# biodatageeks/datafusion-bio-functions

Hardware: AMD Instinct MI355X
Metric: overlap-pairs/sec + probe-rows/sec, IntervalJoinExec 100Mx1M (higher is better)
Workload: dtype int32; 1 GPU; join_100Mx1M_24contigs; probe_rows_per_gpu=100000000, build_rows_per_gpu=1000000, contigs=24, pairs_per_gpu=37210484, parallelism=partition-per-gpu x1, gather=False, build_overlap=True

## Files before the change

datafusion-bio-functions_amd/csrc/ivx_capi.hip:

```cpp
#include "ivx_internal.hpp"
#include <cstdlib>
#include <atomic>
#include <chrono>
#include <cstring>
#include <mutex>
#include <new>
#include <thread>
#include <condition_variable>
#include <deque>


void ivx_ctx::join_tail()
{
    if (!tail_pending) return;
    (void)hipStreamWaitEvent(stream, tail_ev, 0);
    tail_pending = false;
}

ivx_status ivx_ctx::get_scratch(int slot, size_t bytes, void **out)
{
    if (tail_pending && slot != WS_SORTHIST && slot != WS_T0 && slot != WS_T1 && slot != WS_T2) join_tail();
    ivx_buf &b = scratch[slot];
    if (sub_plan.valid && ((sub_plan.slots >> slot) & 1)) sub_plan.valid = false;
    if (join_plan.valid && ((join_plan.rows.slots >> slot) & 1)) join_plan.valid = false;
// ... 191 lines not shown
    *out = nullptr;
    int ndev = 0;
    if (hipGetDeviceCount(&ndev) != hipSuccess || ndev <= 0) return IVX_ERR_NO_DEVICE;
    if (device_ordinal < 0 || device_ordinal >= ndev) return IVX_ERR_NO_DEVICE;
    hipDeviceProp_t prop;
    if (hipGetDeviceProperties(&prop, device_ordinal) != hipSuccess) return IVX_ERR_NO_DEVICE;
    if (std::strncmp(prop.gcnArchName, "gfx950", 6) != 0) return IVX_ERR_NO_DEVICE;
    ivx_ctx *c = new (std::nothrow) ivx_ctx();
    if (!c) return IVX_ERR_OOM;
    c->device = device_ordinal;
    bool ok = hipSetDevice(device_ordinal) == hipSuccess &&
              hipStreamCreateWithFlags(&c->own_stream, hipStreamNonBlocking) == hipSuccess &&
              create_aux_stream(&c->aux) &&
              hipEventCreateWithFlags(&c->ev_fork, hipEventDisableTiming) == hipSuccess &&
              hipEventCreateWithFlags(&c->tail_ev, hipEventDisableTiming) == hipSuccess &&
              hipEventCreate(&c->ev0) == hipSuccess && hipEventCreate(&c->ev1) == hipSuccess &&
              hipMalloc((void **)&c->d_scalars, 64 * sizeof(u64)) == hipSuccess &&
              hipHostMalloc((void **)&c->h_scalars, 64 * sizeof(u64), hipHostMallocDefault) == hipSuccess;
    if (!ok) { ivx_ctx_free(c); return IVX_ERR_HIP; }
    c->stream = c->own_stream;
    if (const char *e = getenv("IVX_BUILD_OVERLAP")) c->overlap = e[0] == '1';
    *out = c;
    return IVX_OK;
}

extern "C" void ivx_ctx_free(ivx_ctx *c)
{
    if (!c) return;
    (void)hipSetDevice(c->device);
    (void)hipStreamSynchronize(c->stream);
    if (c->aux) (void)hipStreamSynchronize(c->aux);
    for (auto &b : c->scratch) if (b.p) (void)hipFree(b.p);
    for (auto &b : c->pinned) if (b.p) (void)hipHostFree(b.p);
    if (c->d_scalars) (void)hipFree(c->d_scalars);
    if (c->h_scalars) (void)hipHostFree(c->h_scalars);
    if (c->ev0) (void)hipEventDestroy(c->ev0);
    if (c->ev1) (void)hipEventDestroy(c->ev1);
    if (c->own_stream) (void)hipStreamDestroy(c->own_stream);
    if (c->aux) (void)hipStreamDestroy(c->aux);
    if (c->ev_fork) (void)hipEventDestroy(c->ev_fork);
    if (c->tail_ev) (void)hipEventDestroy(c->tail_ev);
    delete c;
}

extern "C" const char *ivx_last_error(const ivx_ctx *c) { return c ? c->err.c_str() : "null ctx"; }

extern "C" ivx_status ivx_ctx_set_stream(ivx_ctx *c, void *hip_stream)
{
    if (!c) return IVX_ERR_INVALID;
    if (c->tail_pending) { (void)hipStreamSynchronize(c->aux); c->tail_pending = false; }
    c->stream = (hipStream_t)hip_stream;
    return IVX_OK;
}

extern "C" ivx_status ivx_ctx_use_own_stream(ivx_ctx *c)
{
// ... 107 lines not shown
        }
    }
    if (st == IVX_OK && hipStreamSynchronize(ctx->stream) != hipSuccess) st = ctx->fail(IVX_ERR_HIP, "index build failed on device");
    ctx->building_bytes = 0;
    if (st != IVX_OK) { ivx_index_free(ix); return st; }
    ix->owner_bytes = ctx->live_index_bytes;
    ix->owner_bytes->fetch_add(ix->bytes, std::memory_order_relaxed);
    ctx->metrics.build_mem_used += ix->bytes;
    *out = ix;
    return IVX_OK;
}

extern "C" void ivx_index_free(ivx_index *ix)
{
    if (!ix) return;
    if (ix->ready) { (void)hipEventSynchronize(ix->ready); (void)hipEventDestroy(ix->ready); }
    for (size_t i = 0; i < ix->allocs.size(); i++) pool_give(ix->device, ix->allocs[i], ix->alloc_caps[i]);
    if (ix->owner_bytes) ix->owner_bytes->fetch_sub(ix->bytes, std::memory_order_relaxed);
    delete ix;
}

extern "C" uint64_t ivx_index_rows(const ivx_index *ix) { return ix ? ix->n : 0; }
extern "C" uint64_t ivx_index_device_bytes(const ivx_index *ix) { return ix ? ix->bytes : 0; }

extern "C" ivx_status ivx_index_layout(ivx_ctx *ctx, const ivx_index *ix, uint32_t *out, uint32_t n_out)
{
    if (!ctx) return IVX_ERR_INVALID;
    if (!ix) return ctx->fail(IVX_ERR_INVALID, "null index");
    if (n_out && !out) return ctx->fail(IVX_ERR_INVALID, "null out");
    if (ix->device != ctx->device) return ctx->fail(IVX_ERR_INVALID, "index lives on another device");
    u32 w[IVX_LAYOUT_WORDS] = {};
// ... 726 lines not shown
```

datafusion-bio-functions_amd/csrc/ivx_grid.hip:

```cpp
#include <cstdlib>
#include "ivx_grid.hpp"
#include "ivx_scan.hpp"

namespace {

constexpr int GT = 256;
constexpr u32 KEYS_IN_LDS = 2048;

__global__ void k_init_keystats(i32 *kmin, i32 *kmax, u32 *kcnt, u32 nkeys, ivx_zero_ranges z)
{
    u32 i = blockIdx.x * blockDim.x + threadIdx.x;
    if (i < nkeys) { kmin[i] = INT32_MAX; kmax[i] = INT32_MIN; kcnt[i] = 0; }
    if (blockIdx.x == 0)
        for (int r = 0; r < 3; r++)
            for (u32 j = threadIdx.x; j < z.n[r]; j += blockDim.x) z.p[r][j] = 0;
    for (u32 j = i; j < z.nbig; j += gridDim.x * blockDim.x) z.big[j] = make_uint4(0u, 0u, 0u, 0u);
}

__global__ __launch_bounds__(GT) void k_keystats(const u32 *__restrict__ key, const i32 *__restrict__ v, u64 n,
                                                 u32 nkeys, i32 *kmin, i32 *kmax, u32 *kcnt, u32 *errflag, u32 vs,
                                                 const i32 *__restrict__ vend, u32 *lenhist)
{
    extern __shared__ i32 sh[];
    __shared__ u32 s_len[33];
// ... 1 lines not shown
    const bool priv = nkeys <= KEYS_IN_LDS;
    if (!priv && lenhist) __syncthreads();
    i32 *smin = sh, *smax = sh + nkeys;
    u32 *scnt = (u32 *)(sh + 2 * nkeys);
    if (priv) {
        for (u32 k = threadIdx.x; k < nkeys; k += GT) { smin[k] = INT32_MAX; smax[k] = INT32_MIN; scnt[k] = 0; }
        __syncthreads();
    }
    u32 ck = 0xFFFFFFFFu, ccnt = 0; i32 cmin = INT32_MAX, cmax = INT32_MIN;
    u32 cl = 0xFFFFFFFFu, clcnt = 0;
    auto flush = [&]() {
        if (!ccnt) return;
        if (priv) { atomicMin(&smin[ck], cmin); atomicMax(&smax[ck], cmax); atomicAdd(&scnt[ck], ccnt); }
        else { atomicMin(&kmin[ck], cmin); atomicMax(&kmax[ck], cmax); atomicAdd(&kcnt[ck], ccnt); }
    };
    for (u64 i = (u64)blockIdx.x * GT + threadIdx.x; i < n; i += (u64)gridDim.x * GT) {
        const u32 k = key ? key[i] : 0u;
        if (k >= nkeys) { *errflag = 1; continue; }
        const i32 x = v[i * vs];
        if (lenhist) {
            const i64 len = (i64)vend[i] - (i64)x;
            const u32 c = len <= 0 ? 0u : 64u - (u32)__clzll((u64)len);
            if (c != cl) { if (clcnt) atomicAdd(&s_len[cl], clcnt); cl = c; clcnt = 0; }
            clcnt++;
        }
        if (k != ck) { flush(); ck = k; ccnt = 0; cmin = INT32_MAX; cmax = INT32_MIN; }
        cmin = x < cmin ? x : cmin; cmax = x > cmax ? x : cmax; ccnt++;
    }
    flush();
    if (lenhist && clcnt) atomicAdd(&s_len[cl], clcnt);
    if (priv) {
        __syncthreads();
        for (u32 k = threadIdx.x; k < nkeys; k += GT)
            if (scnt[k]) { atomicMin(&kmin[k], smin[k]); atomicMax(&kmax[k], smax[k]); atomicAdd(&kcnt[k], scnt[k]); }
    }
    if (lenhist) {
        __syncthreads();
        if (threadIdx.x < 33 && s_len[threadIdx.x]) atomicAdd(&lenhist[threadIdx.x], s_len[threadIdx.x]);
    }
}

__global__ __launch_bounds__(GT) void k_keystats_sorted(const u32 *__restrict__ key, const i32 *__restrict__ v, u64 n, u32 nkeys,
// ... 189 lines not shown
```

datafusion-bio-functions_amd/csrc/ivx_internal.hpp:

```cpp
#pragma once
#include <hip/hip_runtime.h>
#include <stdint.h>
#include <atomic>
#include <memory>
#include <string>
#include <vector>
#include "../../include/ivx.h"

typedef uint8_t u8;
typedef uint32_t u32;
typedef int32_t i32;
typedef uint64_t u64;
typedef int64_t i64;

#define IVX_WAVE 64

struct ivx_buf { void *p = nullptr; size_t cap = 0; };

enum { IVX_NSCRATCH = 56, IVX_NPIN = 4 };

struct ivx_sub_plan {
    bool valid = false;
    u64 slots = 0;
    int mem = 0;
// ... 40 lines not shown
    const uint2 *vtab = nullptr;
    const i32 *ds = nullptr, *de = nullptr;
    u32 adj = 0;
    u64 slots = 0;
};

struct ivx_join_plan {
    bool valid = false;
    int mem = 0;
    const void *in[3] = {};
    u64 n = 0;
    u64 total = 0;
    const void *ix = nullptr; u64 ix_serial = 0;
    hipStream_t stream = nullptr;
    ivx_routed rows;
};

struct ivx_ctx {
    int device = 0;
    hipStream_t own_stream = nullptr;
    hipStream_t stream = nullptr;
    hipEvent_t ev0 = nullptr, ev1 = nullptr;
    double last_ms = 0.0;
    std::string err;
    ivx_buf scratch[IVX_NSCRATCH];
    ivx_buf pinned[IVX_NPIN];
    u64 *d_scalars = nullptr;
    u64 *h_scalars = nullptr;
    ivx_sub_plan sub_plan;
    ivx_join_plan join_plan;
    ivx_metrics metrics{};
    u64 mem_limit = 0;
    u64 fill_hint = 0;
    u64 scratch_bytes = 0, building_bytes = 0;
    hipStream_t aux = nullptr;
    hipEvent_t ev_fork = nullptr, tail_ev = nullptr;
    bool overlap = false, tail_pending = false;
    void join_tail();
    std::shared_ptr<std::atomic<u64>> live_index_bytes = std::make_shared<std::atomic<u64>>(0);
    u64 reserved() const { return scratch_bytes + building_bytes + live_index_bytes->load(std::memory_order_relaxed); }

    ivx_status fail(ivx_status st, const std::string &msg) { err = msg; return st; }
    ivx_status fail_hip(const char *what, hipError_t e)
    {
        err = std::string(what) + ": " + hipGetErrorString(e);
        return e == hipErrorOutOfMemory ? IVX_ERR_OOM : IVX_ERR_HIP;
    }
    ivx_status get_scratch(int slot, size_t bytes, void **out);
    ivx_status get_pinned(int slot, size_t bytes, void **out);
};

// ... 96 lines not shown
    int kind = 0;
    int device = 0;
    u64 n = 0;
    u32 nkeys = 0;
    size_t bytes = 0;
    std::shared_ptr<std::atomic<u64>> owner_bytes;
    std::vector<void *> allocs;
    std::vector<size_t> alloc_caps;
    JoinIndexView jv{};
    u32 jv_nreg = 0;
    bool jv_filter = false;
    bool jv_pk24 = false;
    bool jv_fast = false;
    bool jv_fast_unknown = false;
    hipEvent_t ready = nullptr;
    RankGridView gs{}, ge{};
    CoverageView cv{};
    NearestView nv{};
    JoinIndexView nroute{};
    u32 nroute_nreg = 0;
    int flags = 0;
};
enum { IVX_IXF_REGION_ROWVAL = 1 };

ivx_status ivx_scan_exclusive_u32(ivx_ctx *ctx, u32 *data, u64 n, const u32 *skip = nullptr);
ivx_status ivx_scan_exclusive_u64(ivx_ctx *ctx, u64 *data, u64 n);

ivx_status ivx_join_build(ivx_ctx *ctx, ivx_index *ix, const u32 *key, const i32 *s, const i32 *e, u64 n, bool overlap = false);
ivx_status ivx_join_probe(ivx_ctx *ctx, const JoinIndexView &jv, int mode,
                          const u32 *key, const i32 *s, const i32 *e, u64 n,
// ... 22 lines not shown
```

datafusion-bio-functions_amd/csrc/ivx_join.hip:

```cpp
#include <cstdlib>
#include <cstring>
#include "ivx_device.hpp"
#include "ivx_grid.hpp"
#include "ivx_join.hpp"

namespace {

constexpr int BT = 256;

constexpr int LB_T = 1024;
constexpr int LB_ROWS = 4;
constexpr u32 LB_TILE = LB_T * LB_ROWS;
constexpr u32 LB_STRIDE = IVX_MAXREG_WIDE + 1;
constexpr u32 LB_CCAP = 8192;
constexpr u32 LB_MAXTILES = 1024;
constexpr int LB_KEEP = (IVX_RP_ECAP + LB_T - 1) / LB_T;
constexpr u64 LB_MIN_ROWS = 1u << 14, LB_MAX_ROWS = (u64)LB_MAXTILES * LB_TILE;
static_assert(LB_STRIDE == LB_T && LB_TILE <= 4096 && LB_CCAP == (1u << IVX_REG_CS_MAX), "k_lbuild_tiles: one table word per thread, 12-bit ranks");
static inline u32 lb_tstride(u32 ntiles) { return ntiles | 1u; }


__device__ __forceinline__ u32 cells_of(u32 cnt, u32 span, u32 sh) { return cnt ? (sh >= 32 ? 1u : (span >> sh) + 1u) : 0u; }

__global__ __launch_bounds__(1024) void k_join_layout(const i32 *kmin, const i32 *kmax, const u32 *kcnt, u32 nkeys, u64 n,
                                                      i32 *origin, u32 *span, u32 *lbase, u32 *hdr, u64 maxcells,
                                                      u32 *kreg, u32 *rkey, const u32 *lenhist, u32 regmax, u32 *fbase, int filter_mode, int lbuild_ok, const u32 *badkey)
{
    __shared__ u64 red[1024 / IVX_WAVE + 1];
    __shared__ u32 s_sh0;
    const u32 t = threadIdx.x;
    for (u32 k = t; k < nkeys; k += 1024) {
        u32 c = kcnt[k];
        origin[k] = c ? kmin[k] : 0;
        span[k] = c ? (u32)((i64)kmax[k] - (i64)kmin[k]) : 0u;
    }
    __syncthreads();
    __shared__ u64 s_tot[40];
    __shared__ u64 s_loff[IVX_MAXL + 1];
    const u32 wv = t / IVX_WAVE, ln = lane_id();
    constexpr u32 NWV = 1024 / IVX_WAVE;
    const u64 budget0 = 2 * n + nkeys;
    for (u32 sh = IVX_SH_MIN + wv; sh <= 31; sh += NWV) {
        u64 a = 0;
        for (u32 k = ln; k < nkeys; k += IVX_WAVE) a += cells_of(kcnt[k], span[k], sh);
        a = wave_sum(a);
        if (ln == 0) s_tot[sh] = a;
    }
    __syncthreads();
    __shared__ float s_occ0;
    __shared__ u64 s_cum[34];
    __shared__ float s_cost[32], s_cocc[32];
    __shared__ u32 s_shb;
    if (t <= 32) s_cum[t + 1] = lenhist[t];
    __syncthreads();
    __shared__ u32 s_fg;
    if (t == 0) {
        u32 shb = IVX_SH_MIN;
        while (shb < 31 && s_tot[shb] > budget0) shb++;
        s_shb = shb;
        u32 fg = 0xFFFFFFFFu;
        if (filter_mode != 0 && (u64)nkeys * 34 < IVX_FBITS_MAX / 2) {
            u32 g = IVX_SH_MIN;
            while (g < 31 && s_tot[g] + (u64)nkeys * 34 > IVX_FBITS_MAX) g++;
            const double bits = (double)(s_tot[g] + nkeys);
            double touched = 0.0;
            for (u32 b = 0; b <= 32; b++) touched += (double)s_cum[b + 1] * ((b > g ? (double)(3ull << (b - g)) * 0.25 : 0.0) + 1.5);
            if (n && s_tot[g] + (u64)nkeys * 34 <= IVX_FBITS_MAX && (filter_mode == 2 || touched < 0.15 * bits) && touched < 64.0 * (double)n + 1.0e6) fg = g;
        }
        s_fg = fg;
// ... 29 lines not shown
        for (u32 c = 1; c < 32; c++) if (s_cost[c] < s_cost[bi]) bi = c;
#ifdef IVX_SH_BIAS
        { const int b2 = (int)bi + (IVX_SH_BIAS); bi = b2 < 0 ? 0u : (s_shb + (u32)b2 > 31 ? 31 - s_shb : (u32)b2); }
#endif
        s_sh0 = s_shb + bi; s_occ0 = s_cocc[bi];
    }
    __syncthreads();
    const u32 sh0 = s_sh0;
    u32 nlev = 0;
    for (u32 l = 0; l < IVX_MAXL; l++) { nlev = l + 1; if (sh0 + IVX_LSTEP * l >= 32) break; }
    for (u32 l = wv; l < nlev; l += NWV) {
        const u32 sh = sh0 + IVX_LSTEP * l;
        u64 carry = 0;
        for (u32 k0 = 0; k0 < nkeys; k0 += IVX_WAVE) {
            const u32 k = k0 + ln;
            const u64 c = k < nkeys ? cells_of(kcnt[k], span[k], sh) : 0u;
            const u64 inc = wave_incl_scan(c);
            if (k < nkeys) lbase[(u64)l * nkeys + k] = (u32)(carry + inc - c);
            carry += __shfl(inc, IVX_WAVE - 1, IVX_WAVE);
        }
        if (ln == 0) s_tot[l] = carry;
    }
    __syncthreads();
    if (t == 0) {
        u64 run = 0;
        for (u32 l = 0; l < nlev; l++) { s_loff[l] = run; run += s_tot[l]; }
        hdr[HDR_SH0] = sh0;
        hdr[HDR_NLEV] = nlev;
        hdr[HDR_NBINS] = (u32)(run <= maxcells ? run : maxcells);
    }
    __syncthreads();
    for (u32 l = 1 + wv; l < nlev; l += NWV) {
        const u32 add = (u32)s_loff[l];
        for (u32 k = ln; k < nkeys; k += IVX_WAVE) lbase[(u64)l * nkeys + k] += add;
    }
    for (u32 mid = wv; mid <= 32; mid += NWV) {
        u64 a = 0;
        for (u32 k = ln; k < nkeys; k += IVX_WAVE) {
            const u64 c = cells_of(kcnt[k], span[k], sh0);
            a += mid >= 32 ? (c ? 1u : 0u) : ((c + (1ull << mid) - 1) >> mid);
        }
        a = wave_sum(a);
        if (ln == 0) s_tot[mid] = a;
    }
    __syncthreads();
    u32 clo = 0;
    while (clo < 32 && s_tot[clo] > IVX_MAXREG) clo++;
    if (clo > IVX_REG_CS_MAX && clo <= 32 && s_tot[IVX_REG_CS_MAX] <= IVX_MAXREG2) clo = IVX_REG_CS_MAX;
    u64 R = clo < 32 ? (1ull << clo) : 0;
    bool pow2 = true;
    if (clo < 32 && s_occ0 * (float)R > 0.9f * (float)IVX_RP_ECAP) {
        const float want = 0.85f * (float)IVX_RP_ECAP / s_occ0;
        R = want < 1.f ? 1ull : (u64)want;
        pow2 = false;
    }
    auto regions_for = [&](u64 r) -> u64 {
        u64 a = 0;
        for (u32 k = t; k < nkeys; k += 1024) { const u64 c = cells_of(kcnt[k], span[k], sh0); a += (c + r - 1) / r; }
        return block_sum<u64, 1024>(a, red);
    };
    if (R && nkeys > regmax && regions_for(1ull << 40) > regmax) R = 0;
    if (R) {
        if (!(pow2 && clo < 32 && s_tot[clo] <= regmax)) while (regions_for(R) > regmax) { R *= 2; }
        if (!pow2) {
            u64 mc = 0;
            for (u32 k = t; k < nkeys; k += 1024) { const u64 c = cells_of(kcnt[k], span[k], sh0); mc = c > mc ? c : mc; }
            __shared__ u64 s_mc;
            if (t == 0) s_mc = 0;
            __syncthreads();
            atomicMax((unsigned long long *)&s_mc, (unsigned long long)mc);
            __syncthreads();
            const u64 M = ((1ull << 40) + R - 1) / R;
            if (s_mc * R >= (1ull << 40) || s_mc > (1ull << 63) / M || (R & (R - 1)) == 0) {
                u64 p = 1; while (p * 2 <= R) p *= 2;
                R = p; pow2 = true;
                while (regions_for(R) > regmax) R *= 2;
            }
        }
    }
    u32 cs = 32;
    if (R && pow2) { cs = 0; while ((1ull << cs) < R) cs++; }
    u64 rrun = 0;
    for (u32 k0 = 0; k0 < nkeys; k0 += 1024) {
        const u32 k = k0 + t;
        u64 c = k < nkeys ? cells_of(kcnt[k], span[k], sh0) : 0u;
        c = R ? (c + R - 1) / R : 0;
        u64 tot;
        const u64 ex = block_excl_scan<u64, 1024>(c, red, &tot);
        if (k < nkeys && R) {
            kreg[k] = (u32)(rrun + ex);
            for (u64 r = 0; r < c; r++) rkey[rrun + ex + r] = k;
        }
        rrun += tot;
    }
    {
        const u32 fg = s_fg;
        u64 frun = 0;
        for (u32 k0 = 0; k0 < nkeys; k0 += 1024) {
            const u32 k = k0 + t;
            u64 c = (fg != 0xFFFFFFFFu && k < nkeys && kcnt[k]) ? (u64)(((span[k] >> fg) + 2u + 31u) & ~31u) : 0u;
            u64 tot;
            const u64 ex = block_excl_scan<u64, 1024>(c, red, &tot);
            if (k < nkeys) fbase[k] = (u32)(frun + ex);
            frun += tot;
        }
        if (t == 0) { hdr[HDR_FG] = frun <= IVX_FBITS_MAX ? fg : 0xFFFFFFFFu; hdr[HDR_FBITS] = (u32)frun; }
    }
    if (t == 0) {
        kreg[nkeys] = (u32)rrun;
        hdr[HDR_CS] = pow2 ? cs : 0xFFFFFFFFu;
        hdr[HDR_NREG] = R ? (u32)rrun : 0u;
        hdr[HDR_RCELLS] = (u32)(R > 0xFFFFFFFFull ? 0xFFFFFFFFull : R);
        const u64 M = R ? ((1ull << 40) + R - 1) / R : 0;
        hdr[HDR_RMUL_LO] = (u32)M; hdr[HDR_RMUL_HI] = (u32)(M >> 32);
        hdr[HDR_PK24] = (R && sh0 < 24 && R <= (1ull << (24 - sh0))) ? 1u : 0u;
        hdr[HDR_BADKEY] = *badkey;
        hdr[HDR_LBUILD] = (lbuild_ok && R && R <= LB_CCAP && rrun && rrun <= IVX_MAXREG_WIDE && s_cum[33] == s_cum[sh0 + 1]) ? 1u : 0u;
    }
}

__global__ __launch_bounds__(LB_T) void k_lbuild_tiles(const u32 *__restrict__ key, const i32 *__restrict__ s, const i32 *__restrict__ e, u64 n, u32 nkeys,
                                                     const i32 *origin, const u32 *kreg, u32 *hdr, ivx_ent *__restrict__ rows,
                                                     u32 *__restrict__ tab, u32 tstride, u32 *__restrict__ binstart, u64 nbinwords)
{
    if (hdr[HDR_LBUILD] == 0) {
        for (u64 i = (u64)blockIdx.x * LB_T + threadIdx.x; i < nbinwords; i += (u64)gridDim.x * LB_T) binstart[i] = 0;
        return;
    }
    __shared__ u32 s_cnt[LB_STRIDE];
    __shared__ u32 red[LB_T / IVX_WAVE + 1];
    const u32 t = threadIdx.x;
    s_cnt[t] = 0;
// ... 101 lines not shown
        const u32 nlev = hdr[HDR_NLEV], nbins = hdr[HDR_NBINS];
        const u32 l0 = nlev > 1 ? lbase[nkeys] : nbins;
        const u32 len = nbins + 1 - l0, per = (len + nreg - 1) / nreg;
        const u64 a = (u64)l0 + (u64)r * per, b = a + per < (u64)nbins + 1 ? a + per : (u64)nbins + 1;
        for (u64 x = a + t; x < b; x += LB_T) binstart[x] = total;
    }
    __syncthreads();
#pragma unroll
    for (int j = 0; j < LB_KEEP; j++) {
        const u32 i = t + (u32)j * LB_T;
        if (i < N) ent[e0 + atomicAdd(&s_cell[cell_in(mine[j].s)], 1u)] = mine[j];
    }
    for (u32 i = t + LB_KEEP * LB_T; i < N; i += LB_T) { const ivx_ent x = fetch(i); ent[e0 + atomicAdd(&s_cell[cell_in(x.s)], 1u)] = x; }
}

__global__ __launch_bounds__(256) void k_join_regdesc(const i32 *origin, const u32 *span, const u32 *lbase, u32 *hdr,
                                                      const u32 *kreg, const u32 *rkey, const u32 *binstart, ivx_regdesc *rdesc)
{
    const u32 r = threadIdx.x + blockIdx.x * 256;
    if (r == 0) {
        bool upper = hdr[HDR_LEVCNT] == 0;
        for (u32 l = 1; l < hdr[HDR_NLEV]; l++) upper |= hdr[HDR_LEVCNT + l] != 0;
        if (upper) hdr[HDR_SLOW] = 1u;
    }
    if (r >= hdr[HDR_NREG]) return;
    const u32 sh0 = hdr[HDR_SH0];
    const u64 R = hdr[HDR_RCELLS];
    ivx_regdesc d;
    d.k = rkey[r]; d.origin = origin[d.k]; d.span = span[d.k]; d.lb = lbase[d.k];
    const u32 cells0 = (d.span >> sh0) + 1u;
    const u64 rc0w = (u64)(r - kreg[d.k]) * R;
    const u32 rc0 = (u32)rc0w;
    const u64 rc1w = rc0w + R;
    const u32 rc1 = rc1w < cells0 ? (u32)rc1w : cells0;
    d.slo = rc0 ? rc0 - 1u : 0u;
    d.shi = rc1 + IVX_RP_HALO < cells0 ? rc1 + IVX_RP_HALO : cells0;
    d.e0 = binstart[d.lb + d.slo];
    d.ne = binstart[d.lb + d.shi] - d.e0;
    d.rbase = (i32)((i64)d.origin + (i64)(rc0w << sh0));
    if (d.ne > IVX_RP_ECAP || d.shi - d.slo + 1u > 8192u + IVX_RP_HALO + 2u) hdr[HDR_SLOW] = 1u;
// ... 263 lines not shown
    const bool lb_try = n >= LB_MIN_ROWS && n <= LB_MAX_ROWS && !(benv && !strcmp(benv, "global"));
    const u32 lb_tiles = lb_try ? (u32)((n + LB_TILE - 1) / LB_TILE) : 0u;
    IVX_TRY(ctx->get_scratch(WS_GRID2, (n ? n : 1) * (lb_try ? sizeof(ivx_ent) : sizeof(u32)), (void **)&cellid));
    const size_t tabbytes = (size_t)lb_tstride(lb_tiles) * LB_STRIDE * sizeof(u32);
    IVX_TRY(ctx->get_scratch(WS_T9, (n ? n : 1) * sizeof(u32) > tabbytes ? (n ? n : 1) * sizeof(u32) : tabbytes, (void **)&rank));
    errflag = (u32 *)(ctx->d_scalars + 8);
    u32 *lenhist = (u32 *)(ctx->d_scalars + 32);

    ivx_zero_ranges zr{{errflag, lenhist, hdr}, {1u, 34u, (u32)HDR_WORDS}};
    const char *fenv = getenv("IVX_FILTER");
    const int filter_mode = !fenv ? 1 : !strcmp(fenv, "0") ? 0 : !strcmp(fenv, "force") ? 2 : 1;
    static_assert((IVX_FBITS_MAX / 32 + 4) % 4 == 0, "the bitmap is cleared in 16-byte words");
    if (filter_mode) { zr.big = (uint4 *)fbits; zr.nbig = (u32)(fwords / 4); }
    IVX_TRY(ivx_keystats_len(ctx, key, s, n, nkeys, kmin, kmax, kcnt, errflag, 1u, e, lenhist, &zr));
    const u32 grid = ivx_stream_grid(n, BT * 2, 16384);
    hipLaunchKernelGGL(k_join_layout, dim3(1), dim3(1024), 0, st, kmin, kmax, kcnt, nkeys, n, origin, span, lbase, hdr, maxcells, kreg, rkey, (const u32 *)lenhist, (u32)(regcap - 1), fbase, filter_mode, lb_try ? 1 : 0, (const u32 *)errflag);
    if (filter_mode) hipLaunchKernelGGL(k_join_filter, dim3(grid), dim3(BT), 0, st, key, s, e, n, nkeys, (const i32 *)origin, (const u32 *)span, (const u32 *)fbase, (const u32 *)hdr, fbits);
    const bool want_route = ix->kind == IVX_KIND_OVERLAP && n >= (4u << 20);
    overlap = overlap && ctx->overlap && ctx->aux != nullptr && !want_route && n >= (1u << 16);
    hipStream_t tail_st = st;
    struct TailGuard {
        ivx_ctx *c; bool armed = false;
        ~TailGuard() { if (armed) (void)hipStreamSynchronize(c->aux); }
    } guard{ctx};
    bool q_lds = lb_try, q_global = true;
    if (overlap) {
        ctx->join_tail();
        IVX_HIP(ctx, hipEventRecord(ctx->ev_fork, st));
        IVX_HIP(ctx, hipStreamWaitEvent(ctx->aux, ctx->ev_fork, 0));
        tail_st = ctx->aux;
        IVX_HIP(ctx, hipMemcpyAsync(ctx->h_scalars + 32, hdr, HDR_WORDS * sizeof(u32), hipMemcpyDeviceToHost, st));
        IVX_HIP(ctx, hipStreamSynchronize(st));
        if (((const u32 *)(ctx->h_scalars + 32))[HDR_BADKEY]) return ctx->fail(IVX_ERR_INVALID, "build key id >= n_keys");
        q_lds = lb_try && ((const u32 *)(ctx->h_scalars + 32))[HDR_LBUILD] != 0;
        q_global = !q_lds;
        guard.armed = true;
    }
    if (q_lds)
        hipLaunchKernelGGL(k_lbuild_tiles, dim3(lb_tiles), dim3(LB_T), 0, tail_st, key, s, e, n, nkeys, (const i32 *)origin, (const u32 *)kreg, hdr,
                           (ivx_ent *)cellid, rank, lb_tstride(lb_tiles), binstart, maxcells + 1);
    else
        IVX_HIP(ctx, hipMemsetAsync(binstart, 0, (maxcells + 1) * sizeof(u32), tail_st));
    if (q_global) {
        hipLaunchKernelGGL(k_join_count, dim3(grid), dim3(BT), 0, tail_st, key, s, e, n, nkeys, origin, lbase, hdr, binstart, cellid, rank);
        const hipStream_t keep = ctx->stream;
        ctx->stream = tail_st;
        const ivx_status sst = ivx_scan_exclusive_u32(ctx, binstart, maxcells + 1, hdr + HDR_LBUILD);
        ctx->stream = keep;
        IVX_TRY(sst);
        hipLaunchKernelGGL(k_join_scatter, dim3(grid), dim3(BT), 0, tail_st, s, e, n, (const u32 *)binstart, (const u32 *)cellid, (const u32 *)rank, ent, (const u32 *)hdr);
    }
    if (q_lds) {
        const u32 rgrid = regcap - 1 < IVX_MAXREG_WIDE ? (u32)(regcap - 1) : (u32)IVX_MAXREG_WIDE;
        hipLaunchKernelGGL(k_lbuild_regions, dim3(rgrid), dim3(LB_T), 0, tail_st, (const i32 *)origin, (const u32 *)span, (const u32 *)lbase, (const u32 *)kreg,
                           (const u32 *)rkey, (const u32 *)hdr, nkeys, (const ivx_ent *)cellid, (const u32 *)rank, lb_tiles, lb_tstride(lb_tiles), binstart, ent);
    }
    hipLaunchKernelGGL(k_join_regdesc, dim3((u32)((regcap + 255) / 256)), dim3(256), 0, tail_st, origin, span, lbase, hdr, kreg, rkey, binstart, rdesc);
    IVX_HIP(ctx, hipGetLastError());
    if (overlap) {
        if (ix->ready == nullptr) IVX_HIP(ctx, hipEventCreateWithFlags(&ix->ready, hipEventDisableTiming));
        IVX_HIP(ctx, hipEventRecord(ix->ready, ctx->aux));
        IVX_HIP(ctx, hipEventRecord(ctx->tail_ev, ctx->aux));
        ctx->tail_pending = true;
        ix->jv_fast_unknown = true;
    }
    if (want_route) IVX_TRY(ivx_route_view_build(ctx, ix, origin, span, kcnt));

    if (!overlap) {
        IVX_HIP(ctx, hipMemcpyAsync(ctx->h_scalars + 32, hdr, HDR_WORDS * sizeof(u32), hipMemcpyDeviceToHost, st));
        IVX_HIP(ctx, hipStreamSynchronize(st));
    }
    if (((const u32 *)(ctx->h_scalars + 32))[HDR_BADKEY]) return ctx->fail(IVX_ERR_INVALID, "build key id >= n_keys");
    ix->jv_nreg = ((const u32 *)(ctx->h_scalars + 32))[HDR_NREG];
    ix->jv_filter = ((const u32 *)(ctx->h_scalars + 32))[HDR_FG] != 0xFFFFFFFFu;
    ix->jv_pk24 = ((const u32 *)(ctx->h_scalars + 32))[HDR_PK24] != 0;
    ix->jv_fast = ((const u32 *)(ctx->h_scalars + 32))[HDR_SLOW] == 0 && ix->jv_nreg > 0;
    if (want_route) ivx_route_view_ready(ctx, ix);
    guard.armed = false;

    ix->jv.origin = origin; ix->jv.span = span; ix->jv.kcnt = kcnt; ix->jv.lbase = lbase;
    ix->jv.binstart = binstart; ix->jv.ent = ent; ix->jv.hdr = hdr; ix->jv.nkeys = nkeys;
    ix->jv.kreg = kreg; ix->jv.rkey = rkey; ix->jv.rdesc = rdesc;
    ix->jv.fbits = fbits; ix->jv.fbase = fbase;
    return IVX_OK;
}

ivx_status ivx_join_probe(ivx_ctx *ctx, const JoinIndexView &jv, int mode,
                          const u32 *key, const i32 *s, const i32 *e, u64 n,
                          u32 *per_row, u8 *exists, u32 *ob, u32 *op, u64 cap, u64 *d_cursor)
{
    if (n == 0) return IVX_OK;
// ... 18 lines not shown
```

datafusion-bio-functions_amd/csrc/ivx_regions_probe.hip:

```cpp
#include "ivx_regions.hpp"

namespace {


#ifndef IVX_RP_B
#define IVX_RP_B 8
#endif
#ifndef IVX_RP_RING
#define IVX_RP_RING 512
#endif
#ifndef IVX_RP_ECAP
#define IVX_RP_ECAP 6144
#endif
constexpr int RP_B = IVX_RP_B;
constexpr u32 RP_HALO = IVX_RP_HALO;
constexpr u32 RP_CCAP = 8192 + RP_HALO + 2;
constexpr u32 RP_ECAP = IVX_RP_ECAP;
constexpr u32 RP_RING = IVX_RP_RING;
constexpr u32 RP_NSLOT = 4;
constexpr u32 RP_NPG = 64;
constexpr u32 RP_GRID = 256;
#ifndef IVX_RP_VGRID
#define IVX_RP_VGRID 512
#endif
// ... 640 lines not shown
    const u32 sh0 = ix.hdr[HDR_SH0], nlev = ix.hdr[HDR_NLEV];
    auto rows64 = [&](bool ok, u32 r, u32 v) {
        i32 qs = 0, qe = -1; u32 row = 0, k = 0;
        if (ok) {
            u32 pg = pt.ptab[(u64)r * pt.pstride + (v >> pt.lgpg)];
            if (pg == 0u) { pg = 1u; atomicOr((unsigned int *)(cursor + 1), 1u); }
            pg -= 1u;
            const u64 x = pool[((u64)pg << pt.lgpg) + (v & pmask)];
            const u32 lo32 = (u32)x, hi32 = (u32)(x >> 32);
            const u32 len = (lo32 >> 24) | ((rowbits < 32 ? (hi32 >> rowbits) & 0xFFu : 0u) << 8);
            row = hi32 & rowmask;
            k = ix.rkey[r];
            if (len == maxlen) { qs = ps_in[row]; qe = pe_in[row]; }
            else { qs = (i32)((u32)ix.rdesc[r].rbase + (lo32 & 0xFFFFFFu)); qe = (i32)((u32)qs + len); }
        }
        u32 m = 0;
        if (ok) walk(ix, sh0, 0, nlev, k, qs, qe, [&](u32) { m++; });
        const u32 inc = wave_incl_scan(m);
        const u32 tot = __shfl(inc, IVX_WAVE - 1, IVX_WAVE);
        if (tot == 0) return;
        unsigned long long g = 0;
        if (ln == 0) g = atomicAdd(cursor, (unsigned long long)tot);
        g = __shfl(g, 0, IVX_WAVE);
        if (g + tot > cap) return;
        u64 at = g + inc - m;
        if (m) walk(ix, sh0, 0, nlev, k, qs, qe, [&](u32 brow) { ob[at] = brow; op[at] = row; at++; });
    };
    const u32 wave = blockIdx.x * wpb + threadIdx.x / IVX_WAVE, nwave = gridDim.x * wpb;
    for (u32 i0 = wave * IVX_WAVE; i0 < nrow; i0 += nwave * IVX_WAVE) {
        const bool ok = i0 + ln < nrow;
        const u64 e = ok ? rest_rows[i0 + ln] : 0ull;
        rows64(ok, (u32)(e >> 32), (u32)e);
    }
    for (u32 b = wave; b < nbat; b += nwave) {
        const FpRest w = rest[b];
        for (u32 t0 = 0; t0 < w.cnt; t0 += IVX_WAVE) rows64(t0 + ln < w.cnt, w.r, w.first + t0 + ln);
    }
}

#ifndef IVX_RV_WPS
#define IVX_RV_WPS 4
// ... 484 lines not shown
```

Measured before the change: 34.26 billion overlap-pairs/s.

## Cut build sync stalls, batch keystats loads, cache join matches, pool events

```diff
diff --git a/datafusion-bio-functions_amd/csrc/ivx_capi.hip b/datafusion-bio-functions_amd/csrc/ivx_capi.hip
--- a/datafusion-bio-functions_amd/csrc/ivx_capi.hip
+++ b/datafusion-bio-functions_amd/csrc/ivx_capi.hip
@@ -229,6 +229,7 @@
               create_aux_stream(&c->aux) &&
               hipEventCreateWithFlags(&c->ev_fork, hipEventDisableTiming) == hipSuccess &&
               hipEventCreateWithFlags(&c->tail_ev, hipEventDisableTiming) == hipSuccess &&
+              hipEventCreateWithFlags(&c->ev_hdr, hipEventDisableTiming) == hipSuccess &&
               hipEventCreate(&c->ev0) == hipSuccess && hipEventCreate(&c->ev1) == hipSuccess &&
               hipMalloc((void **)&c->d_scalars, 64 * sizeof(u64)) == hipSuccess &&
               hipHostMalloc((void **)&c->h_scalars, 64 * sizeof(u64), hipHostMallocDefault) == hipSuccess;
@@ -255,6 +256,8 @@
     if (c->aux) (void)hipStreamDestroy(c->aux);
     if (c->ev_fork) (void)hipEventDestroy(c->ev_fork);
     if (c->tail_ev) (void)hipEventDestroy(c->tail_ev);
+    if (c->ev_hdr) (void)hipEventDestroy(c->ev_hdr);
+    c->events->close();
     delete c;
 }
 
@@ -392,7 +395,10 @@
 extern "C" void ivx_index_free(ivx_index *ix)
 {
     if (!ix) return;
-    if (ix->ready) { (void)hipEventSynchronize(ix->ready); (void)hipEventDestroy(ix->ready); }
+    if (ix->ready) {
+        (void)hipEventSynchronize(ix->ready);
+        if (ix->events) ix->events->give(ix->ready); else (void)hipEventDestroy(ix->ready);
+    }
     for (size_t i = 0; i < ix->allocs.size(); i++) pool_give(ix->device, ix->allocs[i], ix->alloc_caps[i]);
     if (ix->owner_bytes) ix->owner_bytes->fetch_sub(ix->bytes, std::memory_order_relaxed);
     delete ix;
diff --git a/datafusion-bio-functions_amd/csrc/ivx_grid.hip b/datafusion-bio-functions_amd/csrc/ivx_grid.hip
--- a/datafusion-bio-functions_amd/csrc/ivx_grid.hip
+++ b/datafusion-bio-functions_amd/csrc/ivx_grid.hip
@@ -6,6 +6,7 @@
 
 constexpr int GT = 256;
 constexpr u32 KEYS_IN_LDS = 2048;
+constexpr int KS_ROWS = 8;
 
 __global__ void k_init_keystats(i32 *kmin, i32 *kmax, u32 *kcnt, u32 nkeys, ivx_zero_ranges z)
 {
@@ -39,18 +40,32 @@
         if (priv) { atomicMin(&smin[ck], cmin); atomicMax(&smax[ck], cmax); atomicAdd(&scnt[ck], ccnt); }
         else { atomicMin(&kmin[ck], cmin); atomicMax(&kmax[ck], cmax); atomicAdd(&kcnt[ck], ccnt); }
     };
-    for (u64 i = (u64)blockIdx.x * GT + threadIdx.x; i < n; i += (u64)gridDim.x * GT) {
-        const u32 k = key ? key[i] : 0u;
-        if (k >= nkeys) { *errflag = 1; continue; }
-        const i32 x = v[i * vs];
-        if (lenhist) {
-            const i64 len = (i64)vend[i] - (i64)x;
-            const u32 c = len <= 0 ? 0u : 64u - (u32)__clzll((u64)len);
-            if (c != cl) { if (clcnt) atomicAdd(&s_len[cl], clcnt); cl = c; clcnt = 0; }
-            clcnt++;
-        }
-        if (k != ck) { flush(); ck = k; ccnt = 0; cmin = INT32_MAX; cmax = INT32_MIN; }
-        cmin = x < cmin ? x : cmin; cmax = x > cmax ? x : cmax; ccnt++;
+    const u64 stride = (u64)gridDim.x * GT;
+    for (u64 i0 = (u64)blockIdx.x * GT + threadIdx.x; i0 < n; i0 += KS_ROWS * stride) {
+        u32 rk[KS_ROWS]; i32 rx[KS_ROWS], re[KS_ROWS];
+#pragma unroll
+        for (int j = 0; j < KS_ROWS; j++) {
+            const u64 i = i0 + (u64)j * stride;
+            const bool ok = i < n;
+            rk[j] = ok && key ? key[i] : 0u;
+            rx[j] = ok ? v[i * vs] : 0;
+            re[j] = ok && lenhist ? vend[i] : 0;
+        }
+#pragma unroll
+        for (int j = 0; j < KS_ROWS; j++) {
+            if (i0 + (u64)j * stride >= n) break;
+            const u32 k = rk[j];
+            if (k >= nkeys) { *errflag = 1; continue; }
+            const i32 x = rx[j];
+            if (lenhist) {
+                const i64 len = (i64)re[j] - (i64)x;
+                const u32 c = len <= 0 ? 0u : 64u - (u32)__clzll((u64)len);
+                if (c != cl) { if (clcnt) atomicAdd(&s_len[cl], clcnt); cl = c; clcnt = 0; }
+                clcnt++;
+            }
+            if (k != ck) { flush(); ck = k; ccnt = 0; cmin = INT32_MAX; cmax = INT32_MIN; }
+            cmin = x < cmin ? x : cmin; cmax = x > cmax ? x : cmax; ccnt++;
+        }
     }
     flush();
     if (lenhist && clcnt) atomicAdd(&s_len[cl], clcnt);
diff --git a/datafusion-bio-functions_amd/csrc/ivx_internal.hpp b/datafusion-bio-functions_amd/csrc/ivx_internal.hpp
--- a/datafusion-bio-functions_amd/csrc/ivx_internal.hpp
+++ b/datafusion-bio-functions_amd/csrc/ivx_internal.hpp
@@ -3,6 +3,7 @@
 #include <stdint.h>
 #include <atomic>
 #include <memory>
+#include <mutex>
 #include <string>
 #include <vector>
 #include "../../include/ivx.h"
@@ -78,6 +79,34 @@
     const void *ix = nullptr; u64 ix_serial = 0;
     hipStream_t stream = nullptr;
     ivx_routed rows;
+};
+
+struct ivx_event_pool {
+    std::mutex mu;
+    std::vector<hipEvent_t> free;
+    bool closed = false;
+    hipError_t take(hipEvent_t *out)
+    {
+        {
+            std::lock_guard<std::mutex> lk(mu);
+            if (!free.empty()) { *out = free.back(); free.pop_back(); return hipSuccess; }
+        }
+        return hipEventCreateWithFlags(out, hipEventDisableTiming);
+    }
+    void give(hipEvent_t ev)
+    {
+        {
+            std::lock_guard<std::mutex> lk(mu);
+            if (!closed && free.size() < 8) { free.push_back(ev); return; }
+        }
+        (void)hipEventDestroy(ev);
+    }
+    void close()
+    {
+        std::vector<hipEvent_t> drop;
+        { std::lock_guard<std::mutex> lk(mu); closed = true; drop.swap(free); }
+        for (hipEvent_t ev : drop) (void)hipEventDestroy(ev);
+    }
 };
 
 struct ivx_ctx {
@@ -99,6 +128,8 @@
     u64 scratch_bytes = 0, building_bytes = 0;
     hipStream_t aux = nullptr;
     hipEvent_t ev_fork = nullptr, tail_ev = nullptr;
+    hipEvent_t ev_hdr = nullptr;
+    std::shared_ptr<ivx_event_pool> events = std::make_shared<ivx_event_pool>();
     bool overlap = false, tail_pending = false;
     void join_tail();
     std::shared_ptr<std::atomic<u64>> live_index_bytes = std::make_shared<std::atomic<u64>>(0);
@@ -225,6 +256,7 @@
     bool jv_fast = false;
     bool jv_fast_unknown = false;
     hipEvent_t ready = nullptr;
+    std::shared_ptr<ivx_event_pool> events;
     RankGridView gs{}, ge{};
     CoverageView cv{};
     NearestView nv{};
diff --git a/datafusion-bio-functions_amd/csrc/ivx_join.hip b/datafusion-bio-functions_amd/csrc/ivx_join.hip
--- a/datafusion-bio-functions_amd/csrc/ivx_join.hip
+++ b/datafusion-bio-functions_amd/csrc/ivx_join.hip
@@ -7,6 +7,7 @@
 namespace {
 
 constexpr int BT = 256;
+constexpr u32 LAYOUT_KEYS = 1024;
 
 constexpr int LB_T = 1024;
 constexpr int LB_ROWS = 4;
@@ -24,17 +25,25 @@
 
 __global__ __launch_bounds__(1024) void k_join_layout(const i32 *kmin, const i32 *kmax, const u32 *kcnt, u32 nkeys, u64 n,
                                                       i32 *origin, u32 *span, u32 *lbase, u32 *hdr, u64 maxcells,
-                                                      u32 *kreg, u32 *rkey, const u32 *lenhist, u32 regmax, u32 *fbase, int filter_mode, int lbuild_ok, const u32 *badkey)
+                                                      u32 *kreg, u32 *rkey, const u32 *lenhist, u32 regmax, u32 *fbase, int filter_mode, int lbuild_ok, const u32 *badkey,
+                                                      u32 *hosthdr)
 {
     __shared__ u64 red[1024 / IVX_WAVE + 1];
     __shared__ u32 s_sh0;
     const u32 t = threadIdx.x;
+    __shared__ u32 s_kc[LAYOUT_KEYS], s_sp[LAYOUT_KEYS];
+    __shared__ u64 s_cum[34];
+    const bool keys_in_lds = nkeys <= LAYOUT_KEYS;
     for (u32 k = t; k < nkeys; k += 1024) {
-        u32 c = kcnt[k];
+        const u32 c = kcnt[k];
+        const u32 w = c ? (u32)((i64)kmax[k] - (i64)kmin[k]) : 0u;
         origin[k] = c ? kmin[k] : 0;
-        span[k] = c ? (u32)((i64)kmax[k] - (i64)kmin[k]) : 0u;
-    }
-    __syncthreads();
+        span[k] = w;
+        if (keys_in_lds) { s_kc[k] = c; s_sp[k] = w; }
+    }
+    if (t <= 32) s_cum[t + 1] = lenhist[t];
+    __syncthreads();
+    const u32 *const kc = keys_in_lds ? s_kc : kcnt, *const sp = keys_in_lds ? s_sp : span;
     __shared__ u64 s_tot[40];
     __shared__ u64 s_loff[IVX_MAXL + 1];
     const u32 wv = t / IVX_WAVE, ln = lane_id();
@@ -42,17 +51,14 @@
     const u64 budget0 = 2 * n + nkeys;
     for (u32 sh = IVX_SH_MIN + wv; sh <= 31; sh += NWV) {
         u64 a = 0;
-        for (u32 k = ln; k < nkeys; k += IVX_WAVE) a += cells_of(kcnt[k], span[k], sh);
+        for (u32 k = ln; k < nkeys; k += IVX_WAVE) a += cells_of(kc[k], sp[k], sh);
         a = wave_sum(a);
         if (ln == 0) s_tot[sh] = a;
     }
     __syncthreads();
     __shared__ float s_occ0;
-    __shared__ u64 s_cum[34];
     __shared__ float s_cost[32], s_cocc[32];
     __shared__ u32 s_shb;
-    if (t <= 32) s_cum[t + 1] = lenhist[t];
-    __syncthreads();
     __shared__ u32 s_fg;
     if (t == 0) {
         u32 shb = IVX_SH_MIN;
@@ -112,7 +118,7 @@
         u64 carry = 0;
         for (u32 k0 = 0; k0 < nkeys; k0 += IVX_WAVE) {
             const u32 k = k0 + ln;
-            const u64 c = k < nkeys ? cells_of(kcnt[k], span[k], sh) : 0u;
+            const u64 c = k < nkeys ? cells_of(kc[k], sp[k], sh) : 0u;
             const u64 inc = wave_incl_scan(c);
             if (k < nkeys) lbase[(u64)l * nkeys + k] = (u32)(carry + inc - c);
             carry += __shfl(inc, IVX_WAVE - 1, IVX_WAVE);
@@ -135,7 +141,7 @@
     for (u32 mid = wv; mid <= 32; mid += NWV) {
         u64 a = 0;
         for (u32 k = ln; k < nkeys; k += IVX_WAVE) {
-            const u64 c = cells_of(kcnt[k], span[k], sh0);
+            const u64 c = cells_of(kc[k], sp[k], sh0);
             a += mid >= 32 ? (c ? 1u : 0u) : ((c + (1ull << mid) - 1) >> mid);
         }
         a = wave_sum(a);
@@ -154,7 +160,7 @@
     }
     auto regions_for = [&](u64 r) -> u64 {
         u64 a = 0;
-        for (u32 k = t; k < nkeys; k += 1024) { const u64 c = cells_of(kcnt[k], span[k], sh0); a += (c + r - 1) / r; }
+        for (u32 k = t; k < nkeys; k += 1024) { const u64 c = cells_of(kc[k], sp[k], sh0); a += (c + r - 1) / r; }
         return block_sum<u64, 1024>(a, red);
     };
     if (R && nkeys > regmax && regions_for(1ull << 40) > regmax) R = 0;
@@ -162,7 +168,7 @@
         if (!(pow2 && clo < 32 && s_tot[clo] <= regmax)) while (regions_for(R) > regmax) { R *= 2; }
         if (!pow2) {
             u64 mc = 0;
-            for (u32 k = t; k < nkeys; k += 1024) { const u64 c = cells_of(kcnt[k], span[k], sh0); mc = c > mc ? c : mc; }
+            for (u32 k = t; k < nkeys; k += 1024) { const u64 c = cells_of(kc[k], sp[k], sh0); mc = c > mc ? c : mc; }
             __shared__ u64 s_mc;
             if (t == 0) s_mc = 0;
             __syncthreads();
@@ -181,7 +187,7 @@
     u64 rrun = 0;
     for (u32 k0 = 0; k0 < nkeys; k0 += 1024) {
         const u32 k = k0 + t;
-        u64 c = k < nkeys ? cells_of(kcnt[k], span[k], sh0) : 0u;
+        u64 c = k < nkeys ? cells_of(kc[k], sp[k], sh0) : 0u;
         c = R ? (c + R - 1) / R : 0;
         u64 tot;
         const u64 ex = block_excl_scan<u64, 1024>(c, red, &tot);
@@ -196,7 +202,7 @@
         u64 frun = 0;
         for (u32 k0 = 0; k0 < nkeys; k0 += 1024) {
             const u32 k = k0 + t;
-            u64 c = (fg != 0xFFFFFFFFu && k < nkeys && kcnt[k]) ? (u64)(((span[k] >> fg) + 2u + 31u) & ~31u) : 0u;
+            u64 c = (fg != 0xFFFFFFFFu && k < nkeys && kc[k]) ? (u64)(((sp[k] >> fg) + 2u + 31u) & ~31u) : 0u;
             u64 tot;
             const u64 ex = block_excl_scan<u64, 1024>(c, red, &tot);
             if (k < nkeys) fbase[k] = (u32)(frun + ex);
@@ -214,6 +220,10 @@
         hdr[HDR_PK24] = (R && sh0 < 24 && R <= (1ull << (24 - sh0))) ? 1u : 0u;
         hdr[HDR_BADKEY] = *badkey;
         hdr[HDR_LBUILD] = (lbuild_ok && R && R <= LB_CCAP && rrun && rrun <= IVX_MAXREG_WIDE && s_cum[33] == s_cum[sh0 + 1]) ? 1u : 0u;
+        if (hosthdr) {
+            for (u32 w = 0; w < HDR_WORDS; w++) hosthdr[w] = hdr[w];
+            __threadfence_system();
+        }
     }
 }
 
@@ -345,8 +355,12 @@
     for (u32 i = t + LB_KEEP * LB_T; i < N; i += LB_T) { const ivx_ent x = fetch(i); ent[e0 + atomicAdd(&s_cell[cell_in(x.s)], 1u)] = x; }
 }
 
+__device__ __forceinline__ void regdesc_of(u32 r, const i32 *origin, const u32 *span, const u32 *lbase, u32 *hdr,
+                                           const u32 *kreg, const u32 *rkey, const u32 *binstart, ivx_regdesc *rdesc);
+
 __global__ __launch_bounds__(256) void k_join_regdesc(const i32 *origin, const u32 *span, const u32 *lbase, u32 *hdr,
-                                                      const u32 *kreg, const u32 *rkey, const u32 *binstart, ivx_regdesc *rdesc)
+                                                      const u32 *kreg, const u32 *rkey, const u32 *binstart, ivx_regdesc *rdesc,
+                                                      u32 *hosthdr, u32 *ticket)
 {
     const u32 r = threadIdx.x + blockIdx.x * 256;
     if (r == 0) {
@@ -354,7 +368,23 @@
         for (u32 l = 1; l < hdr[HDR_NLEV]; l++) upper |= hdr[HDR_LEVCNT + l] != 0;
         if (upper) hdr[HDR_SLOW] = 1u;
     }
-    if (r >= hdr[HDR_NREG]) return;
+    if (r < hdr[HDR_NREG]) regdesc_of(r, origin, span, lbase, hdr, kreg, rkey, binstart, rdesc);
+    if (hosthdr == nullptr) return;
+    __shared__ u32 s_last;
+    asm volatile("s_waitcnt vmcnt(0)" ::: "memory");
+    __syncthreads();
+    if (threadIdx.x == 0) { __threadfence(); s_last = atomicAdd(ticket, 1u) == gridDim.x - 1u ? 1u : 0u; }
+    __syncthreads();
+    if (s_last && threadIdx.x == 0) {
+        __threadfence();
+        for (u32 w = 0; w < HDR_WORDS; w++) hosthdr[w] = __hip_atomic_load(&hdr[w], __ATOMIC_RELAXED, __HIP_MEMORY_SCOPE_AGENT);
+        __threadfence_system();
+    }
+}
+
+__device__ __forceinline__ void regdesc_of(u32 r, const i32 *origin, const u32 *span, const u32 *lbase, u32 *hdr,
+                                           const u32 *kreg, const u32 *rkey, const u32 *binstart, ivx_regdesc *rdesc)
+{
     const u32 sh0 = hdr[HDR_SH0];
     const u64 R = hdr[HDR_RCELLS];
     ivx_regdesc d;
@@ -648,26 +678,25 @@
     if (filter_mode) { zr.big = (uint4 *)fbits; zr.nbig = (u32)(fwords / 4); }
     IVX_TRY(ivx_keystats_len(ctx, key, s, n, nkeys, kmin, kmax, kcnt, errflag, 1u, e, lenhist, &zr));
     const u32 grid = ivx_stream_grid(n, BT * 2, 16384);
-    hipLaunchKernelGGL(k_join_layout, dim3(1), dim3(1024), 0, st, kmin, kmax, kcnt, nkeys, n, origin, span, lbase, hdr, maxcells, kreg, rkey, (const u32 *)lenhist, (u32)(regcap - 1), fbase, filter_mode, lb_try ? 1 : 0, (const u32 *)errflag);
-    if (filter_mode) hipLaunchKernelGGL(k_join_filter, dim3(grid), dim3(BT), 0, st, key, s, e, n, nkeys, (const i32 *)origin, (const u32 *)span, (const u32 *)fbase, (const u32 *)hdr, fbits);
     const bool want_route = ix->kind == IVX_KIND_OVERLAP && n >= (4u << 20);
     overlap = overlap && ctx->overlap && ctx->aux != nullptr && !want_route && n >= (1u << 16);
+    u32 *const hosthdr = (u32 *)(ctx->h_scalars + 32);
+    const volatile u32 *const hh = hosthdr;
+    hipLaunchKernelGGL(k_join_layout, dim3(1), dim3(1024), 0, st, kmin, kmax, kcnt, nkeys, n, origin, span, lbase, hdr, maxcells, kreg, rkey, (const u32 *)lenhist, (u32)(regcap - 1), fbase, filter_mode, lb_try ? 1 : 0, (const u32 *)errflag,
+                       overlap ? hosthdr : (u32 *)nullptr);
+    if (overlap) IVX_HIP(ctx, hipEventRecord(ctx->ev_hdr, st));
+    if (filter_mode) hipLaunchKernelGGL(k_join_filter, dim3(grid), dim3(BT), 0, st, key, s, e, n, nkeys, (const i32 *)origin, (const u32 *)span, (const u32 *)fbase, (const u32 *)hdr, fbits);
     hipStream_t tail_st = st;
     struct TailGuard {
         ivx_ctx *c; bool armed = false;
         ~TailGuard() { if (armed) (void)hipStreamSynchronize(c->aux); }
     } guard{ctx};
-    bool q_lds = lb_try, q_global = true;
+    const bool q_lds = lb_try;
     if (overlap) {
         ctx->join_tail();
         IVX_HIP(ctx, hipEventRecord(ctx->ev_fork, st));
         IVX_HIP(ctx, hipStreamWaitEvent(ctx->aux, ctx->ev_fork, 0));
         tail_st = ctx->aux;
-        IVX_HIP(ctx, hipMemcpyAsync(ctx->h_scalars + 32, hdr, HDR_WORDS * sizeof(u32), hipMemcpyDeviceToHost, st));
-        IVX_HIP(ctx, hipStreamSynchronize(st));
-        if (((const u32 *)(ctx->h_scalars + 32))[HDR_BADKEY]) return ctx->fail(IVX_ERR_INVALID, "build key id >= n_keys");
-        q_lds = lb_try && ((const u32 *)(ctx->h_scalars + 32))[HDR_LBUILD] != 0;
-        q_global = !q_lds;
         guard.armed = true;
     }
     if (q_lds)
@@ -675,7 +704,7 @@
                            (ivx_ent *)cellid, rank, lb_tstride(lb_tiles), binstart, maxcells + 1);
     else
         IVX_HIP(ctx, hipMemsetAsync(binstart, 0, (maxcells + 1) * sizeof(u32), tail_st));
-    if (q_global) {
+    {
         hipLaunchKernelGGL(k_join_count, dim3(grid), dim3(BT), 0, tail_st, key, s, e, n, nkeys, origin, lbase, hdr, binstart, cellid, rank);
         const hipStream_t keep = ctx->stream;
         ctx->stream = tail_st;
@@ -689,10 +718,14 @@
         hipLaunchKernelGGL(k_lbuild_regions, dim3(rgrid), dim3(LB_T), 0, tail_st, (const i32 *)origin, (const u32 *)span, (const u32 *)lbase, (const u32 *)kreg,
                            (const u32 *)rkey, (const u32 *)hdr, nkeys, (const ivx_ent *)cellid, (const u32 *)rank, lb_tiles, lb_tstride(lb_tiles), binstart, ent);
     }
-    hipLaunchKernelGGL(k_join_regdesc, dim3((u32)((regcap + 255) / 256)), dim3(256), 0, tail_st, origin, span, lbase, hdr, kreg, rkey, binstart, rdesc);
+    hipLaunchKernelGGL(k_join_regdesc, dim3((u32)((regcap + 255) / 256)), dim3(256), 0, tail_st, origin, span, lbase, hdr, kreg, rkey, binstart, rdesc,
+                       overlap ? (u32 *)nullptr : hosthdr, lenhist + 33);
     IVX_HIP(ctx, hipGetLastError());
     if (overlap) {
-        if (ix->ready == nullptr) IVX_HIP(ctx, hipEventCreateWithFlags(&ix->ready, hipEventDisableTiming));
+        if (ix->ready == nullptr) {
+            ix->events = ctx->events;
+            IVX_HIP(ctx, ctx->events->take(&ix->ready));
+        }
         IVX_HIP(ctx, hipEventRecord(ix->ready, ctx->aux));
         IVX_HIP(ctx, hipEventRecord(ctx->tail_ev, ctx->aux));
         ctx->tail_pending = true;
@@ -700,15 +733,13 @@
     }
     if (want_route) IVX_TRY(ivx_route_view_build(ctx, ix, origin, span, kcnt));
 
-    if (!overlap) {
-        IVX_HIP(ctx, hipMemcpyAsync(ctx->h_scalars + 32, hdr, HDR_WORDS * sizeof(u32), hipMemcpyDeviceToHost, st));
-        IVX_HIP(ctx, hipStreamSynchronize(st));
-    }
-    if (((const u32 *)(ctx->h_scalars + 32))[HDR_BADKEY]) return ctx->fail(IVX_ERR_INVALID, "build key id >= n_keys");
-    ix->jv_nreg = ((const u32 *)(ctx->h_scalars + 32))[HDR_NREG];
-    ix->jv_filter = ((const u32 *)(ctx->h_scalars + 32))[HDR_FG] != 0xFFFFFFFFu;
-    ix->jv_pk24 = ((const u32 *)(ctx->h_scalars + 32))[HDR_PK24] != 0;
-    ix->jv_fast = ((const u32 *)(ctx->h_scalars + 32))[HDR_SLOW] == 0 && ix->jv_nreg > 0;
+    if (overlap) IVX_HIP(ctx, hipEventSynchronize(ctx->ev_hdr));
+    else IVX_HIP(ctx, hipStreamSynchronize(st));
+    if (hh[HDR_BADKEY]) return ctx->fail(IVX_ERR_INVALID, "build key id >= n_keys");
+    ix->jv_nreg = hh[HDR_NREG];
+    ix->jv_filter = hh[HDR_FG] != 0xFFFFFFFFu;
+    ix->jv_pk24 = hh[HDR_PK24] != 0;
+    ix->jv_fast = hh[HDR_SLOW] == 0 && ix->jv_nreg > 0;
     if (want_route) ivx_route_view_ready(ctx, ix);
     guard.armed = false;
 
diff --git a/datafusion-bio-functions_amd/csrc/ivx_regions_probe.hip b/datafusion-bio-functions_amd/csrc/ivx_regions_probe.hip
--- a/datafusion-bio-functions_amd/csrc/ivx_regions_probe.hip
+++ b/datafusion-bio-functions_amd/csrc/ivx_regions_probe.hip
@@ -678,8 +678,11 @@
             if (len == maxlen) { qs = ps_in[row]; qe = pe_in[row]; }
             else { qs = (i32)((u32)ix.rdesc[r].rbase + (lo32 & 0xFFFFFFu)); qe = (i32)((u32)qs + len); }
         }
-        u32 m = 0;
-        if (ok) walk(ix, sh0, 0, nlev, k, qs, qe, [&](u32) { m++; });
+        u32 m = 0, a0 = 0, a1 = 0;
+        if (ok) walk(ix, sh0, 0, nlev, k, qs, qe, [&](u32 brow) {
+            if (m == 0) a0 = brow; else if (m == 1) a1 = brow;
+            m++;
+        });
         const u32 inc = wave_incl_scan(m);
         const u32 tot = __shfl(inc, IVX_WAVE - 1, IVX_WAVE);
         if (tot == 0) return;
@@ -688,7 +691,11 @@
         g = __shfl(g, 0, IVX_WAVE);
         if (g + tot > cap) return;
         u64 at = g + inc - m;
-        if (m) walk(ix, sh0, 0, nlev, k, qs, qe, [&](u32 brow) { ob[at] = brow; op[at] = row; at++; });
+        if (m == 0) return;
+        if (m <= 2) {
+            ob[at] = a0; op[at] = row;
+            if (m == 2) { ob[at + 1] = a1; op[at + 1] = row; }
+        } else walk(ix, sh0, 0, nlev, k, qs, qe, [&](u32 brow) { ob[at] = brow; op[at] = row; at++; });
     };
     const u32 wave = blockIdx.x * wpb + threadIdx.x / IVX_WAVE, nwave = gridDim.x * wpb;
     for (u32 i0 = wave * IVX_WAVE; i0 < nrow; i0 += nwave * IVX_WAVE) {
```

Result: no change. 34.55 billion overlap-pairs/s, median of 3 (+0.9%).
